# Gaukler/PlainRenderer

Measured on AMD Instinct MI355X. Metric: frames/sec full GI+shade+post @4K; %HBM roofline; 1/2/4/8-GPU scaling, higher is better.
Workload: dtype f32

## Files before the change

### plainrenderer_amd/csrc/backend.cpp

```cpp
#include "backend.h"
#include "kernels_fast/pcf_taps.h"

#include <dlfcn.h>
#include <deque>
#include <algorithm>
#include <chrono>
#include <mutex>
#include <cstdlib>
#include <atomic>
#include <set>
#include <thread>
#include <unordered_map>
#include <unordered_set>
#include <cmath>
#include <cstring>
#include <map>
#include <memory>

#include "../../include/plr.h"

namespace plr {

struct ShaderEntry { std::string name; LaunchFn fn = nullptr; LaunchFn fast = nullptr; };
static bool shaderReadsBindless(const std::string& shader) {
    return shader == "deferredShading.comp" || shader == "sdfDiffuseTrace.comp" || shader == "sdfDebugVisualisation.comp";
}
static bool shaderTakesColumns(const std::string& shader) {
    static const char* const names[] = {"histogramPerTile.comp", "histogramCombineTiles.comp", "depthHiZPyramid.comp", "depthPyramidApex.comp", "depthDownscale.comp",
                                        "sdfCameraTileCulling.comp", "sdfDiffuseTrace.comp", "filterIndirectDiffuseSpatial.comp", "filterIndirectDiffuseTemporal.comp",
                                        "indirectLightUpscale.comp", "deferredShading.comp", "temporalFilter.comp", "bloomDownsample.comp", "bloomUpsample.comp",
                                        "applyBloom.comp", "tonemapping.comp", "giSampleRequests.comp"};
    for (const char* n : names) if (shader == n) return true;
    return false;
}
static bool storageBindingIsReadOnly(const std::string& shader, uint32_t binding) { return shader == "lightMatrix.comp" && binding == 1; }
static std::deque<ShaderEntry>& registry() {
    static std::deque<ShaderEntry> r;
    return r;
}
static std::mutex& registryMutex() {
    static std::mutex m;
    return m;
}
ShaderRegistrar::ShaderRegistrar(const char* name, LaunchFn fn, bool fast) {
    std::lock_guard<std::mutex> lock(registryMutex());
    for (auto& e : registry())
        if (e.name == name) { (fast ? e.fast : e.fn) = fn; return; }
    ShaderEntry e;
    e.name = name;
    (fast ? e.fast : e.fn) = fn;
    registry().push_back(e);
}

struct FusionEntry {
    std::string label;
    std::vector<std::string> shaders;
    FusedLaunchFn fn;
    bool writesSignatures = false;
// ... 1377 lines not shown
        for (size_t k = 0; k < plan.count; k++) { prepareCtx(g->executions[plan.group + k], g->earlyStream, globalPtr); ctxs[k] = &g->executions[plan.group + k].ctx; }
        hipStream_t previous = g->curStream;
        g->curStream = g->earlyStream;
        if (timed) {
            std::string name;
            for (size_t k = 0; k < plan.count; k++) name += (k ? " + " : "") + g->passes[g->executions[plan.group + k].pass]->name;
            name += " (" + plan.f->earlyLabel + ", early stream)";
            if (int trc = beginSegment(g->fusedNames.insert(name).first->c_str())) return trc;
        }
        EarlyPart part;
        part.mode = EarlyPart::Launch;
        const int rc = plan.f->early(ctxs, plan.count, part);
        if (rc) { g_err = "early part of fused launch '" + plan.f->label + "': " + g_err; return rc < 0 ? rc : PLR_ERR_HIP; }
        if (timed) if (int trc = endSegment()) return trc;
        g->curStream = previous;
        if (int erc = orderEvent(&plan.done)) return erc;
        HIP_TRY(hipEventRecord(plan.done, g->earlyStream));
        plan.launched = true;
        g->lastEarly++;
    }
    return PLR_OK;
}

static int tryFusedLaunch(size_t i, size_t last, hipStream_t stream, const GlobalUbo* globalPtr, bool timed, size_t* covered) {
    *covered = 0;
    if (!g->fusion || g->mathMode != PLR_MATH_FAST) return PLR_OK;
    for (const FusionEntry& f : fusions()) {
        const size_t n = f.shaders.size();
        if (i + n > last) continue;
        if (g->debugSig && !f.writesSignatures) continue;
        bool match = true;
        for (size_t k = 0; k < n && match; k++) match = g->passes[g->executions[i + k].pass]->shader == f.shaders[k];
        for (size_t k = 0; k < n && match; k++) match = !g->executions[i + k].edgesFirst();
        if (!match) continue;
        const PassCtx* ctxs[8];
        if (n > 8) continue;
        for (size_t k = 0; k < n; k++) { prepareCtx(g->executions[i + k], stream, globalPtr); ctxs[k] = &g->executions[i + k].ctx; }
        EarlyPlan* early = nullptr;
        for (EarlyPlan& plan : g_earlyPlans) if (plan.launched && plan.group == i && plan.f == &f) early = &plan;
        if (early) {
            HIP_TRY(hipStreamWaitEvent(stream, early->done, 0));
            for (size_t k = 0; k < n; k++) g->executions[i + k].ctx.earlyPartDone = true;
        }
        if (g->fusion >= 2) {
            for (size_t k = 0; k < n; k++) {
                Execution& x = g->executions[i + k];
                for (int b = 0; b < kMaxBindings; b++) {
                    if (!x.ctx.hasStorage(b)) continue;
                    const void* key = nullptr;
                    for (const Access& a : x.access) if (a.write && a.key == x.ctx.storage[b].ptr) key = a.key;
                    if (!key) continue;
                    bool outside = false;
                    for (size_t j = 0; j < g->executions.size() && !outside; j++) {
                        if (j >= i && j < i + n) continue;
                        for (const Access& a : g->executions[j].access) if (a.key == key) { outside = true; break; }
                    }
                    if (!outside) x.ctx.elidableStorage |= 1u << b;
                }
            }
        }
        const char* label = nullptr;
        g->curStream = stream;
        if (timed) {
            std::string name;
            for (size_t k = 0; k < n; k++) name += (k ? " + " : "") + g->passes[g->executions[i + k].pass]->name;
            label = g->fusedNames.insert(name).first->c_str();
            if (int trc = beginSegment(label)) return trc;
        }
        g->currentPassName = label ? label : f.label.c_str();
        for (size_t k = 0; k < n; k++) touchAccesses(g->executions[i + k].access);
        Execution& first = g->executions[i];
        first.ctx.pendingFillSlot = nullptr; first.ctx.pendingFillsTaken = false; first.ctx.applyPendingFillsNow = nullptr;
        if (g->pendingFillSlot) {
            if (f.takesFills && stream == g->stream) { first.ctx.pendingFillSlot = g->pendingFillSlot; first.ctx.applyPendingFillsNow = &applyPendingFillsNow; }
            else if (int frc = applyPendingFillsNow()) return frc;
        }
        for (size_t k = 0; k < n; k++) if (int src = refuseStaleReads(g->executions[i + k], &g->executions[i], n)) return src;
        const int rc = f.fn(ctxs, n);
// ... 678 lines not shown
```

### plainrenderer_amd/csrc/device/image.h

```cpp
#pragma once
#include "vecmath.h"

namespace plr {

enum Format : int32_t {
    F_R8 = 0, F_RG8 = 1, F_RGBA8 = 2, F_R16F = 3, F_RG16F = 4, F_RG32F = 5, F_RG16SN = 6, F_RGBA16F = 7,
    F_RGBA16SN = 8, F_RGBA32F = 9, F_R11G11B10 = 10, F_D16 = 11, F_D32 = 12, F_BC1 = 13, F_BC3 = 14, F_BC5 = 15,
    F_BGRA8 = 16
};

struct ImgView {
    void* ptr;
    int32_t w, h, d;
    int32_t fmt;
};

PLR_DI float halfBitsToFloat(uint32_t h) {
    union { uint16_t u; _Float16 f; } c;
    c.u = (uint16_t)h;
    return (float)c.f;
}
PLR_DI uint32_t floatToHalfBits(float v) {
#ifndef PLR_FAST_SET
    asm volatile("" : "+v"(v));
// ... 18 lines not shown
    const uint32_t subnormal = f2u(v + magic) - f2u(magic);
    uint32_t r = v < 6.103515625e-05f ? subnormal : normal;
    r = r < maxFinite ? r : maxFinite;
    r = u == 0x7f800000u ? expMax : r;
    r = (u >> 31) ? 0u : r;
    r = (u & 0x7fffffffu) > 0x7f800000u ? (expMax | (1u << (M - 1))) : r;
    return r;
}

PLR_DI uint32_t packR11G11B10Exact(vec3 c) {
    return encodeUFloat<6>(c.x) | (encodeUFloat<6>(c.y) << 11) | (encodeUFloat<5>(c.z) << 22);
}

template <int M> PLR_DI uint32_t encodeUFloatInRange(float v) {
    constexpr int shift = 23 - M;
    const uint32_t s = f2u(v * 1.92592994438723585e-34f);
    return (s + ((1u << (shift - 1)) - 1u) + ((s >> shift) & 1u)) >> shift;
}
constexpr uint32_t kUFloatInRangeLimit = 0x477d0000u;
__device__ __attribute__((noinline)) inline uint32_t packR11G11B10OutOfRange(float x, float y, float z) { return packR11G11B10Exact(vec3(x, y, z)); }
PLR_DI uint32_t packR11G11B10Fast(vec3 c) {
    const uint32_t top = max(max(f2u(c.x), f2u(c.y)), f2u(c.z));
    if (__builtin_amdgcn_ballot_w64(top >= kUFloatInRangeLimit) != 0ull) return packR11G11B10OutOfRange(c.x, c.y, c.z);
    return encodeUFloatInRange<6>(c.x) | (encodeUFloatInRange<6>(c.y) << 11) | (encodeUFloatInRange<5>(c.z) << 22);
}

PLR_DI uint32_t packR11G11B10(vec3 c) {
#ifdef PLR_FAST_SET
    return packR11G11B10Fast(c);
#else
    return packR11G11B10Exact(c);
#endif
}

PLR_DI float decodeUnorm8(uint32_t c) { return (float)c / 255.0f; }
PLR_DI float decodeUnorm8Newton(uint32_t c) {
    const float x = (float)c, r = 0x1.010102p-8f, q = x * r;
    return __builtin_fmaf(__builtin_fmaf(-255.f, q, x), r, q);
}
PLR_DI uint32_t encodeUnorm8(float v) {
    if (v != v) return 0u;
    return (uint32_t)__float2int_rn(gclamp(v, 0.f, 1.f) * 255.0f);
}
PLR_DI float decodeSnorm16(int32_t c) { return gmax((float)c / 32767.0f, -1.0f); }
PLR_DI float decodeUnorm16(uint32_t c) { return (float)c / 65535.0f; }

// ... 175 lines not shown
```

### plainrenderer_amd/csrc/kernels_fast/bloom_fast.hip

```cpp
#include "../backend.h"
#include "../device/shading_common.h"
#include <cstdlib>

namespace plr {
namespace fastbloom {

constexpr int TW = 64, TH = 16;
constexpr int ROWS_A = 16, ROWS_B = 12;

struct Tap { int i0, i1; float w0, w1; };

PLR_DI Tap tap1D(float u, int n, float h) {
    int i0; float a;
    linearCoord(u * (float)n, &i0, &a);
    Tap t;
    t.i0 = clampi(i0, n); t.i1 = clampi(i0 + 1, n);
    t.w0 = (1.f - a) * h; t.w1 = a * h;
    return t;
}

template <bool LOWEST>
PLR_DI void bloomUpsampleFastBlock(ImgView source, ImgView previous, ImgView target, float blurRadius, int coverW, int coverH, int yBase, int xBase, unsigned bx, unsigned by) {
    __shared__ float HA[ROWS_A][3][TW];
    __shared__ float HB[ROWS_B][3][TW];
// ... 143 lines not shown
    uint32_t* out = (uint32_t*)target.ptr;
#pragma unroll
    for (int q = 0; q < QY; q++)
#pragma unroll
        for (int py = 0; py < 2; py++) {
            const int y = Y + 2 * q + py;
            if (y >= coverH || y < yBase) continue;
            uint32_t* orow = out + (size_t)y * (size_t)target.w + X;
            const uint32_t p0 = packR11G11B10(acc[q][py][0]), p1 = packR11G11B10(acc[q][py][1]);
            if (X + 1 < coverW) *(uint2*)orow = make_uint2(p0, p1);
            else orow[0] = p0;
        }
}
template <int QY>
__global__ __launch_bounds__(256) void bloomUpsampleQuadKernel(ImgView source, ImgView previous, ImgView target, ParityWeights pw, bool lowest, int coverW, int coverH,
                                                               int yBase, int xBase) { bloomUpsampleQuadBlock<QY>(source, previous, target, pw, lowest, coverW, coverH, yBase, xBase, blockIdx.x, blockIdx.y); }

constexpr int kStripCols = 60, kStripRows = 8;
PLR_DI float laneLeft(float v) { return __builtin_bit_cast(float, __builtin_amdgcn_mov_dpp(__builtin_bit_cast(int, v), 0x138, 0xf, 0xf, true)); }
PLR_DI float laneRight(float v) { return __builtin_bit_cast(float, __builtin_amdgcn_mov_dpp(__builtin_bit_cast(int, v), 0x130, 0xf, 0xf, true)); }
PLR_DI vec3 laneLeft(const vec3& v) { return vec3(laneLeft(v.x), laneLeft(v.y), laneLeft(v.z)); }
PLR_DI vec3 laneRight(const vec3& v) { return vec3(laneRight(v.x), laneRight(v.y), laneRight(v.z)); }

template <bool LOWEST>
__global__ __launch_bounds__(256) void bloomUpsampleStripKernel(ImgView source, ImgView previous, ImgView target, ParityWeights pw, int coverW, int coverH, int yBase, int xBase) {
    const int lane = (int)(threadIdx.x & 63u), wave = (int)(threadIdx.x >> 6);
    const int kc = (xBase >> 1) + (int)blockIdx.x * kStripCols - 2 + lane;
    const int m0 = (yBase >> 1) + ((int)blockIdx.y * 4 + wave) * kStripRows;
    if (2 * m0 >= coverH) return;
    float wt[2][5], wb[2][3];
#pragma unroll
    for (int p = 0; p < 2; p++) {
#pragma unroll
        for (int j = 0; j < 5; j++) { wt[p][j] = pw.tent[p][j]; asm volatile("" : "+v"(wt[p][j])); }
#pragma unroll
        for (int j = 0; j < 3; j++) { wb[p][j] = pw.box[p][j]; asm volatile("" : "+v"(wb[p][j])); }
    }
    const int sw = source.w, sh = source.h;
    const uint32_t* src = (const uint32_t*)source.ptr + clampi(kc, sw);
    uint32_t ta[kStripRows + 4], tb[kStripRows + 2];
#pragma unroll
    for (int r = 0; r < kStripRows + 4; r++) ta[r] = src[(size_t)clampi(m0 - 2 + r, sh) * (size_t)sw];
    if (!LOWEST) {
        const int pwid = previous.w, phei = previous.h;
        const uint32_t* prv = (const uint32_t*)previous.ptr + clampi(kc, pwid);
#pragma unroll
        for (int r = 0; r < kStripRows + 2; r++) tb[r] = prv[(size_t)clampi(m0 - 1 + r, phei) * (size_t)pwid];
    }
    vec3 h0[kStripRows + 4], h1[kStripRows + 4], g0[kStripRows + 2], g1[kStripRows + 2];
    auto tentRow = [&](int r) {
        const vec3 c2 = unpackR11G11B10(ta[r]);
        const vec3 c1 = laneLeft(c2), c0 = laneLeft(c1), c3 = laneRight(c2), c4 = laneRight(c3);
        vec3 a(0.f), b(0.f);
        a = a + c0 * wt[0][0]; b = b + c0 * wt[1][0];
        a = a + c1 * wt[0][1]; b = b + c1 * wt[1][1];
        a = a + c2 * wt[0][2]; b = b + c2 * wt[1][2];
        a = a + c3 * wt[0][3]; b = b + c3 * wt[1][3];
        a = a + c4 * wt[0][4]; b = b + c4 * wt[1][4];
        h0[r] = a; h1[r] = b;
    };
    auto boxRow = [&](int r) {
        const vec3 c1 = unpackR11G11B10(tb[r]);
        const vec3 c0 = laneLeft(c1), c2 = laneRight(c1);
        vec3 a(0.f), b(0.f);
        a = a + c0 * wb[0][0]; b = b + c0 * wb[1][0];
        a = a + c1 * wb[0][1]; b = b + c1 * wb[1][1];
        a = a + c2 * wb[0][2]; b = b + c2 * wb[1][2];
        g0[r] = a; g1[r] = b;
    };
#pragma unroll
    for (int r = 0; r < 4; r++) tentRow(r);
    if (!LOWEST) {
#pragma unroll
        for (int r = 0; r < 2; r++) boxRow(r);
    }
    const bool outputLane = lane >= 2 && lane < 2 + kStripCols && 2 * kc < coverW;
    const bool both = 2 * kc + 1 < coverW;
    uint32_t* out = (uint32_t*)target.ptr + 2 * kc;
#pragma unroll
    for (int q = 0; q < kStripRows; q++) {
        tentRow(q + 4);
        if (!LOWEST) boxRow(q + 2);
#pragma unroll
        for (int py = 0; py < 2; py++) {
            vec3 a(0.f), b(0.f);
#pragma unroll
            for (int j = 0; j < 5; j++) { a = a + h0[q + j] * wt[py][j]; b = b + h1[q + j] * wt[py][j]; }
            if (!LOWEST) {
#pragma unroll
                for (int j = 0; j < 3; j++) { a = a + g0[q + j] * wb[py][j]; b = b + g1[q + j] * wb[py][j]; }
            }
            const int y = 2 * (m0 + q) + py;
            if (y < coverH && outputLane) {
                uint32_t* orow = out + (size_t)y * (size_t)target.w;
                const uint32_t p0 = packR11G11B10(a), p1 = packR11G11B10(b);
                if (both) *(uint2*)orow = make_uint2(p0, p1);
                else orow[0] = p0;
            }
        }
    }
}

static bool accumulateTap(float position, float weight, int base, int n, float* w) {
    const float sane = std::min(std::max(position, -1.0e6f), 1.0e6f);
    const int ti = (int)std::floor((sane - 0.5f) * 256.0f + 0.5f);
    const int i0 = ti >> 8;
    const float a = (float)(ti & 255) * (1.0f / 256.0f);
    const int j0 = i0 - base, j1 = i0 + 1 - base;
    if ((1.f - a) != 0.f) { if (j0 < 0 || j0 >= n) return false; w[j0] += weight * (1.f - a); }
    if (a != 0.f) { if (j1 < 0 || j1 >= n) return false; w[j1] += weight * a; }
    return true;
}

static bool makeParityWeights(float blurRadius, ParityWeights* pw) {
    const int k = 8;
    for (int p = 0; p < 2; p++) {
        const float s = (float)k + 0.25f + 0.5f * (float)p;
        for (float& v : pw->tent[p]) v = 0.f;
        for (float& v : pw->box[p]) v = 0.f;
        bool ok = accumulateTap(s, 0.5f, k - 2, 5, pw->tent[p]) && accumulateTap(s + blurRadius, 0.25f, k - 2, 5, pw->tent[p]) &&
                  accumulateTap(s - blurRadius, 0.25f, k - 2, 5, pw->tent[p]) && accumulateTap(s + 0.5f, 0.5f, k - 1, 3, pw->box[p]) &&
                  accumulateTap(s - 0.5f, 0.5f, k - 1, 3, pw->box[p]);
        if (!ok) return false;
// ... 49 lines not shown
    p.gridX = divUp((unsigned)(w - x0), (unsigned)TW); p.gridY = divUp((unsigned)(h - yBase), (unsigned)TH);
    return 0;
}

static int launch(const PassCtx& c) {
    UpPlan p;
    if (int rc = planUp(c, &p)) return rc;
    const dim3 grid(p.gridX, p.gridY);
    switch (p.kind) {
        case UP_NOTHING: return 0;
        case UP_STRIP:
            if (p.lowest) bloomUpsampleStripKernel<true><<<grid, 256, 0, c.stream>>>(p.source, p.source, p.target, p.pw, p.w, p.h, p.yBase, p.x0);
            else bloomUpsampleStripKernel<false><<<grid, 256, 0, c.stream>>>(p.source, p.previous, p.target, p.pw, p.w, p.h, p.yBase, p.x0);
            break;
        case UP_QUAD: bloomUpsampleQuadKernel<kQuadQY><<<grid, 256, 0, c.stream>>>(p.source, p.previous, p.target, p.pw, p.lowest != 0, p.w, p.h, p.yBase, p.x0); break;
        default:
            if (p.lowest) bloomUpsampleFastKernel<true><<<grid, 256, 0, c.stream>>>(p.source, p.source, p.target, p.blurRadius, p.w, p.h, p.yBase, p.x0);
            else bloomUpsampleFastKernel<false><<<grid, 256, 0, c.stream>>>(p.source, p.previous, p.target, p.blurRadius, p.w, p.h, p.yBase, p.x0);
    }
    PLR_CHECK_LAUNCH(c);
    return 0;
}

PLR_DI void bloomDownsampleFastBlock(ImgView source, ImgView target, int coverW, int coverH, int yBase, int xBase, unsigned bx, unsigned by) {
    const int k = (xBase >> 1) + (int)(bx * 64u + (threadIdx.x & 63u));
    const int m = (yBase >> 1) + (int)(by * 4u + (threadIdx.x >> 6));
    const int X = 2 * k, Y = 2 * m;
    if (X >= coverW || Y >= coverH) return;
    const uint32_t* src = (const uint32_t*)source.ptr;
    const int sx = 4 * k - 1;
    const bool interior = sx >= 0 && sx + 5 < source.w;
    vec3 centre[2][2], border[2][2];
#pragma unroll
    for (int i = 0; i < 4; i++) { centre[i >> 1][i & 1] = vec3(0.f); border[i >> 1][i & 1] = vec3(0.f); }
#pragma unroll
    for (int r = 0; r < 6; r++) {
        const uint32_t* row = src + (size_t)clampi(4 * m - 1 + r, source.h) * (size_t)source.w;
        uint32_t t[6];
        if (interior) {
            uint4 v; uint2 u;
            __builtin_memcpy(&v, row + sx, 16);
            __builtin_memcpy(&u, row + sx + 4, 8);
            t[0] = v.x; t[1] = v.y; t[2] = v.z; t[3] = v.w; t[4] = u.x; t[5] = u.y;
        } else { for (int c = 0; c < 6; c++) t[c] = row[clampi(sx + c, source.w)]; }
        vec3 col[6];
#pragma unroll
// ... 199 lines not shown
            L.source = d.source; L.previous = d.source; L.target = d.target; L.blurRadius = 0.f; L.lowest = 0;
            L.w = d.w; L.h = d.h; L.yBase = d.y0; L.x0 = d.x0; L.kind = d.kind; L.gridX = d.gridX; L.tiles = d.gridX * d.gridY;
        }
        if (L.tiles == 0 || (int)L.tiles > chainMaxTiles()) return kUseGeneralKernel;
        if (i > 0 && L.source.ptr != cp.level[i - 1].target.ptr) return kUseGeneralKernel;
        maxTiles = std::max(maxTiles, L.tiles);
    }
    const PassCtx& c = *ctxs[0];
    cp.counters = (uint32_t*)c.scratch(64);
    if (!cp.counters) return kUseGeneralKernel;
    unsigned grid = 0;
    if (int rc = chainGrid<UP>(c, maxTiles, &grid)) return rc;
    bloomChainKernel<UP><<<grid, 256, 0, c.stream>>>(cp);
    PLR_CHECK_LAUNCH(c);
    return 0;
}

}

static int fastbloom_up_launch(const PassCtx& c) { return fastbloom::launch(c); }
PLR_REGISTER_SHADER_FAST("bloomUpsample.comp", fastbloom_up_launch);
static int fastbloom_down_launch(const PassCtx& c) { return fastbloom::launchDown(c); }
PLR_REGISTER_SHADER_FAST("bloomDownsample.comp", fastbloom_down_launch);
static int fastbloom_down_chain(const PassCtx* const* ctxs, size_t count) { return fastbloom::launchChain<false>(ctxs, count); }
static int fastbloom_up_chain(const PassCtx* const* ctxs, size_t count) { return fastbloom::launchChain<true>(ctxs, count); }
static int fastbloom_down_chain4(const PassCtx* const* ctxs, size_t count) { return fastbloom_down_chain(ctxs, count); }
static int fastbloom_down_chain3(const PassCtx* const* ctxs, size_t count) { return fastbloom_down_chain(ctxs, count); }
static int fastbloom_down_chain2(const PassCtx* const* ctxs, size_t count) { return fastbloom_down_chain(ctxs, count); }
static int fastbloom_up_chain4(const PassCtx* const* ctxs, size_t count) { return fastbloom_up_chain(ctxs, count); }
static int fastbloom_up_chain3(const PassCtx* const* ctxs, size_t count) { return fastbloom_up_chain(ctxs, count); }
static int fastbloom_up_chain2(const PassCtx* const* ctxs, size_t count) { return fastbloom_up_chain(ctxs, count); }
PLR_REGISTER_FUSION("bloomDownsample x4 (persistent chain)", fastbloom_down_chain4, "bloomDownsample.comp", "bloomDownsample.comp", "bloomDownsample.comp", "bloomDownsample.comp");
PLR_REGISTER_FUSION("bloomDownsample x3 (persistent chain)", fastbloom_down_chain3, "bloomDownsample.comp", "bloomDownsample.comp", "bloomDownsample.comp");
PLR_REGISTER_FUSION("bloomDownsample x2 (persistent chain)", fastbloom_down_chain2, "bloomDownsample.comp", "bloomDownsample.comp");
PLR_REGISTER_FUSION("bloomUpsample x4 (persistent chain)", fastbloom_up_chain4, "bloomUpsample.comp", "bloomUpsample.comp", "bloomUpsample.comp", "bloomUpsample.comp");
PLR_REGISTER_FUSION("bloomUpsample x3 (persistent chain)", fastbloom_up_chain3, "bloomUpsample.comp", "bloomUpsample.comp", "bloomUpsample.comp");
PLR_REGISTER_FUSION("bloomUpsample x2 (persistent chain)", fastbloom_up_chain2, "bloomUpsample.comp", "bloomUpsample.comp");
}
```

### plainrenderer_amd/csrc/kernels_fast/gi_spatial_fast.hip

```cpp
#include "../backend.h"
#include "../device/shading_common.h"
#include "../device/xcd.h"
#include "../device/buffer_fetch.h"
#include "fused_gi.h"
#include <cstdlib>
#include <map>
#include <utility>
#include <vector>
#include <type_traits>

namespace plr {

PLR_DI float rcpf(float x) { return __builtin_amdgcn_rcpf(x); }

constexpr int kSampleKeys = 5, kSampleTableFloats = 160;
__global__ void spatialSampleTableKernel(float* __restrict__ table) {
    const int key = (int)threadIdx.x / 32, i = (int)threadIdx.x % 32;
    if (key >= kSampleKeys) return;
    uint32_t rngState = wang_hash((uint32_t)key);
    float r0 = 0.f, r1 = 0.f;
    for (int k = 0; k <= i; k++) { r0 = rand01(rngState); r1 = rand01(rngState); }
    float sn, cs;
    det_sincosf(2.f * PLR_GLSL_PI * r1, &sn, &cs);
    float* t = table + key * kSampleTableFloats;
// ... 32 lines not shown
    if (wi >= words) return;
    uint8_t* bytes = blockIdx.y ? bytes1 : bytes0;
    uint32_t* bitmap = blockIdx.y ? bitmap1 : bitmap0;
    const uint32_t y = wi / rowWords, xw = wi - y * rowWords;
    uint4* src = (uint4*)(bytes + (size_t)y * pitch + (size_t)xw * 32u);
    const uint4 a = src[0], c = src[1];
    const uint32_t d[8] = {a.x, a.y, a.z, a.w, c.x, c.y, c.z, c.w};
    uint32_t bits = 0u;
#pragma unroll
    for (int k = 0; k < 8; k++) {
        const uint32_t v = d[k];
        bits |= (((v & 0xffu) ? 1u : 0u) | ((v & 0xff00u) ? 2u : 0u) | ((v & 0xff0000u) ? 4u : 0u) | ((v & 0xff000000u) ? 8u : 0u)) << (4 * k);
    }
    bitmap[wi] = bits;
    if (bits) { src[0] = make_uint4(0u, 0u, 0u, 0u); src[1] = make_uint4(0u, 0u, 0u, 0u); }
}

struct SpatialFrameConsts {
    float tsx, tsy;
    float dW, dH;
    float nW, nH;
    float3 vpRowNorms;
};
template <int DEPTH_FMT, int TX, bool SAME_GRID, bool PACKED, bool SIG, bool MARK = false>
__global__ __launch_bounds__(256) void spatialFilterFastKernel(ImgView outYSH, ImgView outCoCg, ImgView inYSH, ImgView inCoCg, ImgView depthTexture, ImgView normalTexture,
                                                               const GlobalUbo* __restrict__ g, const float* __restrict__ sampleTables, const uint4* __restrict__ packed, int filterIndex,
                                                               int coverW, int coverH, int yBase, int xBase, int tilesX, int tilesY, int chunkRows, uint32_t* __restrict__ sig,
                                                               uint32_t validY0, uint32_t validRowCount, uint32_t validX0, uint32_t validColCount, int rowMissShrinks,
                                                               SpatialFrameConsts fc, uint32_t* __restrict__ requestBitmap = nullptr, uint32_t bitmapRowWords = 0, int requestPhase = 0,
                                                               uint32_t* __restrict__ requestBitmap2 = nullptr) {
    const float* samples = sampleTables + min(g->frameIndexMod4 + (uint32_t)filterIndex, (uint32_t)(kSampleKeys - 1)) * kSampleTableFloats;
    constexpr int TY = 256 / TX;
    int tileX, tileY;
    if (!xcdWalk2(tilesX, tilesY, chunkRows & 0xffff, chunkRows >> 16, tileX, tileY)) return;
    const int px = xBase + tileX * TX + (int)(threadIdx.x % TX);
    const int py = yBase + tileY * TY + (int)(threadIdx.x / TX);
    if (px >= coverW || py >= coverH) return;

    const float nearP = g->nearPlane, farP = g->farPlane;
    const float nf = nearP * farP, nmf = nearP - farP;
    const vec3 fwd = ld3(g->cameraForward), up = ld3(g->cameraUp), right = ld3(g->cameraRight), camPos = ld3(g->cameraPosition);
    const float tanH = g->cameraTanFovHalf, tanA = g->cameraTanFovHalf * g->cameraAspectRatio;
    const float dW = fc.dW, dH = fc.dH;
    const int dwi = depthTexture.w, dhi = depthTexture.h;

    float radiusWorld = filterIndex == 1 ? 1.f : 1.5f;
    if (MARK || requestPhase != 0) {
        const uint32_t rY0 = MARK ? validY0 : (uint32_t)yBase, rYn = MARK ? validRowCount : (uint32_t)(coverH - yBase);
// ... 481 lines not shown
```

### plainrenderer_amd/csrc/kernels_fast/stream_fast.hip

```cpp
#include "../backend.h"
#include "../device/shading_common.h"
#include "fused_gi.h"
#include "upscale_quad.h"
#include "../device/fastmath.h"

namespace plr {
namespace faststream {

PLR_DI float rcpf(float x) { return __builtin_amdgcn_rcpf(x); }
PLR_DI float clamp01(float x) { return __builtin_amdgcn_fmed3f(x, 0.f, 1.f); }

__global__ __launch_bounds__(256) void applyBloomFastKernel(ImgView target, ImgView bloom, float strength, int coverW, int coverH, int yBase, int xBase) {
    const int x0 = xBase + (int)(blockIdx.x * 64u + (threadIdx.x & 63u)) * 4;
    const int y = yBase + (int)(blockIdx.y * 4u + (threadIdx.x >> 6));
    if (y >= coverH || x0 >= coverW) return;
    uint32_t* trow = (uint32_t*)target.ptr + (size_t)y * (size_t)target.w;
    const uint32_t* brow = (const uint32_t*)bloom.ptr + (size_t)y * (size_t)bloom.w;
    const int n = min(4, coverW - x0);
    uint32_t s[4] = {0u, 0u, 0u, 0u}, b[4] = {0u, 0u, 0u, 0u};
    const bool wide = n == 4 && (target.w & 3) == 0;
    if (wide) {
        const uint4 sv = *(const uint4*)(trow + x0), bv = *(const uint4*)(brow + x0);
        s[0] = sv.x; s[1] = sv.y; s[2] = sv.z; s[3] = sv.w; b[0] = bv.x; b[1] = bv.y; b[2] = bv.z; b[3] = bv.w;
    } else for (int i = 0; i < n; i++) { s[i] = trow[x0 + i]; b[i] = brow[x0 + i]; }
    uint32_t o[4];
#pragma unroll
    for (int i = 0; i < 4; i++) {
        const vec3 sc = unpackR11G11B10(s[i]), bc = unpackR11G11B10(b[i]);
        o[i] = packR11G11B10(sc + (bc - sc) * strength);
    }
    if (wide) *(uint4*)(trow + x0) = make_uint4(o[0], o[1], o[2], o[3]);
    else for (int i = 0; i < n; i++) trow[x0 + i] = o[i];
}

static int launchApplyBloom(const PassCtx& c) {
    if (int rc = c.needStorage(0, F_R11G11B10, "applyBloom target")) return rc;
    if (int rc = c.needSampled(1, F_R11G11B10, "applyBloom bloomTexture")) return rc;
    if (c.push.size() < 4) return c.fail(-1, "applyBloom: push constant bloomStrength missing");
    const ImgView& target = c.storage[0];
    if (c.sampled[1].w != target.w || c.sampled[1].h != target.h) return kUseGeneralKernel;
    float strength;
    std::memcpy(&strength, c.push.data(), 4);
    const PassCtx::RowSpan rs = c.rowSpan(target.h);
    const PassCtx::ColSpan cs = c.colSpan(target.w);
    const int w = cs.x1, x0 = cs.x0, h = rs.y1, y0 = rs.y0;
    if (w <= x0 || h <= y0) return 0;
    applyBloomFastKernel<<<dim3(divUp((unsigned)(w - x0), 256u), divUp((unsigned)(h - y0), 4u)), 256, 0, c.stream>>>(target, c.sampled[1], strength, w, h, y0, x0);
    PLR_CHECK_LAUNCH(c);
    return 0;
}

PLR_DI float srgb(float l) {
    const float hi = __builtin_amdgcn_exp2f((1.0f / 2.4f) * __builtin_amdgcn_logf(fabsf(l))) * 1.055f - 0.055f;
    return l <= 0.0031308f ? l * 12.92f : hi;
}
PLR_DI uint32_t unorm8(float v) { return (uint32_t)__float2int_rn(clamp01(v) * 255.0f); }

template <bool BGRA>
PLR_DI uint32_t tonemapPixel(vec3 c, int x, float time, uint32_t nyA, uint32_t nyB) {
    const uint32_t UI0 = 1597334673u, UI1 = 3812015801u, UI2 = 2798796415u;
    const float UIF = 1.0f / (float)0xffffffffu;
    vec3 v(0.59719f * c.x + 0.35458f * c.y + 0.04823f * c.z, 0.07600f * c.x + 0.90834f * c.y + 0.01566f * c.z, 0.02840f * c.x + 0.13383f * c.y + 0.83777f * c.z);
    const vec3 a = v * (v + 0.0245786f) - 0.000090537f;
    const vec3 b = v * (0.983729f * v + 0.4329510f) + 0.238081f;
    v = vec3(a.x * rcpf(b.x), a.y * rcpf(b.y), a.z * rcpf(b.z));
    const vec3 o(clamp01(1.60475f * v.x + -0.53108f * v.y + -0.07367f * v.z), clamp01(-0.10208f * v.x + 1.10813f * v.y + -0.00605f * v.z),
                 clamp01(-0.00327f * v.x + -0.07276f * v.y + 1.07602f * v.z));
    const uint32_t qxA = (uint32_t)(int32_t)(float)(uint32_t)((float)x * time), qxB = (uint32_t)(int32_t)(float)(uint32_t)(((float)x + 165.f) * time);
    const uint32_t mA = (qxA * UI0) ^ nyA ^ (qxA * UI2), mB = (qxB * UI0) ^ nyB ^ (qxB * UI2);
    const vec3 noise = (vec3((float)(mA * UI0), (float)(mA * UI1), (float)(mA * UI2)) + vec3((float)(mB * UI0), (float)(mB * UI1), (float)(mB * UI2))) * UIF - 1.f;
    const vec3 s = vec3(srgb(o.x), srgb(o.y), srgb(o.z)) + noise * (1.f / 255.f);
    uint32_t p = unorm8(s.z) | (unorm8(s.y) << 8) | (unorm8(s.x) << 16) | (255u << 24);
    if (!BGRA) p = (p & 0xff00ff00u) | ((p >> 16) & 0xffu) | ((p & 0xffu) << 16);
    return p;
}
PLR_DI void tonemapRowTerms(int y, float time, uint32_t* nyA, uint32_t* nyB) {
    const uint32_t UI1 = 3812015801u;
    const uint32_t qyA = (uint32_t)(int32_t)(float)(uint32_t)((float)y * time), qyB = (uint32_t)(int32_t)(float)(uint32_t)(((float)y + 1292.f) * time);
    *nyA = qyA * UI1; *nyB = qyB * UI1;
}

template <bool BGRA>
__global__ __launch_bounds__(256) void tonemappingFastKernel(ImgView src, ImgView dst, const GlobalUbo* __restrict__ g, int coverW, int coverH, int yBase, int xBase) {
    const int x0 = xBase + (int)(blockIdx.x * 64u + (threadIdx.x & 63u)) * 4;
    const int y = yBase + (int)(blockIdx.y * 4u + (threadIdx.x >> 6));
    if (y >= coverH || x0 >= coverW) return;
    const float time = g->time;
    const uint32_t* srow = (const uint32_t*)src.ptr + (size_t)y * (size_t)src.w;
    uint32_t* drow = (uint32_t*)dst.ptr + (size_t)y * (size_t)dst.w;
    const int n = min(4, coverW - x0);
    uint32_t in[4] = {0u, 0u, 0u, 0u}, out[4];
    const bool wide = n == 4 && (src.w & 3) == 0 && (dst.w & 3) == 0;
    if (wide) { const uint4 v = *(const uint4*)(srow + x0); in[0] = v.x; in[1] = v.y; in[2] = v.z; in[3] = v.w; }
    else for (int i = 0; i < n; i++) in[i] = srow[x0 + i];
    uint32_t nyA, nyB;
    tonemapRowTerms(y, time, &nyA, &nyB);
#pragma unroll
    for (int i = 0; i < 4; i++) out[i] = tonemapPixel<BGRA>(unpackR11G11B10(in[i]), x0 + i, time, nyA, nyB);
    if (wide) *(uint4*)(drow + x0) = make_uint4(out[0], out[1], out[2], out[3]);
    else for (int i = 0; i < n; i++) drow[x0 + i] = out[i];
}

template <bool BGRA>
__global__ __launch_bounds__(256) void applyBloomTonemapKernel(ImgView target, ImgView bloom, ImgView dst, const GlobalUbo* __restrict__ g, float strength, int coverW, int coverH, int yBase, int xBase) {
    const int x0 = xBase + (int)(blockIdx.x * 64u + (threadIdx.x & 63u)) * 4;
    const int y = yBase + (int)(blockIdx.y * 4u + (threadIdx.x >> 6));
    if (y >= coverH || x0 >= coverW) return;
    const float time = g->time;
    uint32_t* trow = (uint32_t*)target.ptr + (size_t)y * (size_t)target.w;
    const uint32_t* brow = (const uint32_t*)bloom.ptr + (size_t)y * (size_t)bloom.w;
    uint32_t* drow = (uint32_t*)dst.ptr + (size_t)y * (size_t)dst.w;
    const uint4 sv = *(const uint4*)(trow + x0), bv = *(const uint4*)(brow + x0);
    const uint32_t s[4] = {sv.x, sv.y, sv.z, sv.w}, b[4] = {bv.x, bv.y, bv.z, bv.w};
    uint32_t nyA, nyB;
    tonemapRowTerms(y, time, &nyA, &nyB);
    uint32_t o[4], t[4];
#pragma unroll
    for (int i = 0; i < 4; i++) {
        const vec3 sc = unpackR11G11B10(s[i]), bc = unpackR11G11B10(b[i]);
        o[i] = packR11G11B10(sc + (bc - sc) * strength);
        t[i] = tonemapPixel<BGRA>(unpackR11G11B10(o[i]), x0 + i, time, nyA, nyB);
    }
    *(uint4*)(trow + x0) = make_uint4(o[0], o[1], o[2], o[3]);
    *(uint4*)(drow + x0) = make_uint4(t[0], t[1], t[2], t[3]);
}

static int launchTonemapping(const PassCtx& c) {
    if (int rc = c.needGlobal()) return rc;
    if (int rc = c.needSampled(1, F_R11G11B10, "tonemapping imageIn")) return rc;
    if (int rc = c.needStorage(0, -1, "tonemapping imageOut")) return rc;
    const ImgView& src = c.sampled[1];
    const ImgView& dst = c.storage[0];
    if (dst.fmt != F_BGRA8 && dst.fmt != F_RGBA8) return c.fail(-4, "tonemapping imageOut must be BGRA8_uNorm or RGBA8");
    const PassCtx::ColSpan cs = c.colSpan(std::min(dst.w, src.w));
    const int coverW = cs.x1, xBase = cs.x0;
    const PassCtx::RowSpan rs = c.rowSpan(std::min(dst.h, src.h));
    const int coverH = rs.y1, y0 = rs.y0;
    if (coverW <= xBase || coverH <= y0) return 0;
    const dim3 grid(divUp((unsigned)(coverW - xBase), 256u), divUp((unsigned)(coverH - y0), 4u));
    if (dst.fmt == F_BGRA8) tonemappingFastKernel<true><<<grid, 256, 0, c.stream>>>(src, dst, c.global, coverW, coverH, y0, xBase);
    else tonemappingFastKernel<false><<<grid, 256, 0, c.stream>>>(src, dst, c.global, coverW, coverH, y0, xBase);
    PLR_CHECK_LAUNCH(c);
    return 0;
}

struct Pair8 { uint2 a, b; };
PLR_DI Pair8 loadPairRGBA16F(const ImgView& im, int x0, int x1, int y) {
// ... 377 lines not shown
```

Before: 1426.

## Fuse final bloom upsample with applyBloom and tonemapping into one strip kernel

Adds a fusion that runs the mip-0 bloom upsample, the bloom apply and tonemapping in a single strip kernel. The upsampled bloom is exchanged between lane pairs via DPP and consumed directly, so the full-resolution bloom target write can be skipped when nothing else reads it, which removes one full-res write plus two reads and two launches. Elision analysis now checks per-mip bindings for bloom shaders, and per-column dither terms are precomputed in LDS. The fused kernel carries higher register pressure, pins waves_per_eu and prefetches rows, which could cost occupancy.

```diff
diff --git a/plainrenderer_amd/csrc/backend.cpp b/plainrenderer_amd/csrc/backend.cpp
--- a/plainrenderer_amd/csrc/backend.cpp
+++ b/plainrenderer_amd/csrc/backend.cpp
@@ -34,6 +34,7 @@
     return false;
 }
 static bool storageBindingIsReadOnly(const std::string& shader, uint32_t binding) { return shader == "lightMatrix.comp" && binding == 1; }
+static bool shaderAddressesBoundMipsOnly(const std::string& shader) { return shader == "bloomDownsample.comp" || shader == "bloomUpsample.comp"; }
 static std::deque<ShaderEntry>& registry() {
     static std::deque<ShaderEntry> r;
     return r;
@@ -1457,6 +1458,16 @@
     return PLR_OK;
 }
 
+static bool touchesLevel(const Execution& y, const void* key, const ImgView& level) {
+    bool names = false;
+    for (const Access& a : y.access) names = names || a.key == key;
+    if (!names) return false;
+    if (y.callback || !shaderAddressesBoundMipsOnly(g->passes[y.pass]->shader)) return true;
+    for (int b = 0; b < kMaxBindings; b++)
+        if ((y.ctx.hasSampled(b) && y.ctx.sampled[b].ptr == level.ptr) || (y.ctx.hasStorage(b) && y.ctx.storage[b].ptr == level.ptr)) return true;
+    return false;
+}
+
 static int tryFusedLaunch(size_t i, size_t last, hipStream_t stream, const GlobalUbo* globalPtr, bool timed, size_t* covered) {
     *covered = 0;
     if (!g->fusion || g->mathMode != PLR_MATH_FAST) return PLR_OK;
@@ -1488,7 +1499,7 @@
                     bool outside = false;
                     for (size_t j = 0; j < g->executions.size() && !outside; j++) {
                         if (j >= i && j < i + n) continue;
-                        for (const Access& a : g->executions[j].access) if (a.key == key) { outside = true; break; }
+                        outside = touchesLevel(g->executions[j], key, x.ctx.storage[b]);
                     }
                     if (!outside) x.ctx.elidableStorage |= 1u << b;
                 }
diff --git a/plainrenderer_amd/csrc/device/image.h b/plainrenderer_amd/csrc/device/image.h
--- a/plainrenderer_amd/csrc/device/image.h
+++ b/plainrenderer_amd/csrc/device/image.h
@@ -64,6 +64,11 @@
 PLR_DI uint32_t packR11G11B10Fast(vec3 c) {
     const uint32_t top = max(max(f2u(c.x), f2u(c.y)), f2u(c.z));
     if (__builtin_amdgcn_ballot_w64(top >= kUFloatInRangeLimit) != 0ull) return packR11G11B10OutOfRange(c.x, c.y, c.z);
+    return encodeUFloatInRange<6>(c.x) | (encodeUFloatInRange<6>(c.y) << 11) | (encodeUFloatInRange<5>(c.z) << 22);
+}
+PLR_DI uint32_t packR11G11B10FastInline(vec3 c) {
+    const uint32_t top = max(max(f2u(c.x), f2u(c.y)), f2u(c.z));
+    if (__builtin_expect(__builtin_amdgcn_ballot_w64(top >= kUFloatInRangeLimit) != 0ull, 0)) return packR11G11B10Exact(c);
     return encodeUFloatInRange<6>(c.x) | (encodeUFloatInRange<6>(c.y) << 11) | (encodeUFloatInRange<5>(c.z) << 22);
 }
 
diff --git a/plainrenderer_amd/csrc/kernels_fast/bloom_fast.hip b/plainrenderer_amd/csrc/kernels_fast/bloom_fast.hip
--- a/plainrenderer_amd/csrc/kernels_fast/bloom_fast.hip
+++ b/plainrenderer_amd/csrc/kernels_fast/bloom_fast.hip
@@ -1,5 +1,6 @@
 #include "../backend.h"
 #include "../device/shading_common.h"
+#include "tonemap_pixel.h"
 #include <cstdlib>
 
 namespace plr {
@@ -189,8 +190,17 @@
 PLR_DI vec3 laneLeft(const vec3& v) { return vec3(laneLeft(v.x), laneLeft(v.y), laneLeft(v.z)); }
 PLR_DI vec3 laneRight(const vec3& v) { return vec3(laneRight(v.x), laneRight(v.y), laneRight(v.z)); }
 
-template <bool LOWEST>
-__global__ __launch_bounds__(256) void bloomUpsampleStripKernel(ImgView source, ImgView previous, ImgView target, ParityWeights pw, int coverW, int coverH, int yBase, int xBase) {
+PLR_DI uint32_t lanePartner(uint32_t v) { return (uint32_t)__builtin_amdgcn_mov_dpp((int)v, 0xB1, 0xf, 0xf, true); }
+
+struct StripTail {
+    ImgView scene, dst;
+    const GlobalUbo* global;
+    float strength;
+    int storeLevel;
+};
+
+template <bool LOWEST, int TAIL>
+PLR_DI void bloomUpsampleStripBody(ImgView source, ImgView previous, ImgView target, ParityWeights pw, int coverW, int coverH, int yBase, int xBase, const StripTail& tail) {
     const int lane = (int)(threadIdx.x & 63u), wave = (int)(threadIdx.x >> 6);
     const int kc = (xBase >> 1) + (int)blockIdx.x * kStripCols - 2 + lane;
     const int m0 = (yBase >> 1) + ((int)blockIdx.y * 4 + wave) * kStripRows;
@@ -205,16 +215,21 @@
     }
     const int sw = source.w, sh = source.h;
     const uint32_t* src = (const uint32_t*)source.ptr + clampi(kc, sw);
+    constexpr int kTailAhead = 1;
+    constexpr int aheadA = TAIL ? 4 + kTailAhead : kStripRows + 4, aheadB = TAIL ? 2 + kTailAhead : kStripRows + 2;
     uint32_t ta[kStripRows + 4], tb[kStripRows + 2];
-#pragma unroll
-    for (int r = 0; r < kStripRows + 4; r++) ta[r] = src[(size_t)clampi(m0 - 2 + r, sh) * (size_t)sw];
+    const int pwid = previous.w, phei = previous.h;
+    const uint32_t* prv = (const uint32_t*)previous.ptr + clampi(kc, pwid);
+    auto loadA = [&](int r) { ta[r] = src[(size_t)clampi(m0 - 2 + r, sh) * (size_t)sw]; };
+    auto loadB = [&](int r) { tb[r] = prv[(size_t)clampi(m0 - 1 + r, phei) * (size_t)pwid]; };
+#pragma unroll
+    for (int r = 0; r < aheadA; r++) loadA(r);
     if (!LOWEST) {
-        const int pwid = previous.w, phei = previous.h;
-        const uint32_t* prv = (const uint32_t*)previous.ptr + clampi(kc, pwid);
-#pragma unroll
-        for (int r = 0; r < kStripRows + 2; r++) tb[r] = prv[(size_t)clampi(m0 - 1 + r, phei) * (size_t)pwid];
+#pragma unroll
+        for (int r = 0; r < aheadB; r++) loadB(r);
     }
     vec3 h0[kStripRows + 4], h1[kStripRows + 4], g0[kStripRows + 2], g1[kStripRows + 2];
+    auto pin = [](vec3& a, vec3& b) { asm volatile("" : "+v"(a.x), "+v"(a.y), "+v"(a.z), "+v"(b.x), "+v"(b.y), "+v"(b.z)); };
     auto tentRow = [&](int r) {
         const vec3 c2 = unpackR11G11B10(ta[r]);
         const vec3 c1 = laneLeft(c2), c0 = laneLeft(c1), c3 = laneRight(c2), c4 = laneRight(c3);
@@ -224,6 +239,7 @@
         a = a + c2 * wt[0][2]; b = b + c2 * wt[1][2];
         a = a + c3 * wt[0][3]; b = b + c3 * wt[1][3];
         a = a + c4 * wt[0][4]; b = b + c4 * wt[1][4];
+        if (TAIL) pin(a, b);
         h0[r] = a; h1[r] = b;
     };
     auto boxRow = [&](int r) {
@@ -233,6 +249,7 @@
         a = a + c0 * wb[0][0]; b = b + c0 * wb[1][0];
         a = a + c1 * wb[0][1]; b = b + c1 * wb[1][1];
         a = a + c2 * wb[0][2]; b = b + c2 * wb[1][2];
+        if (TAIL) pin(a, b);
         g0[r] = a; g1[r] = b;
     };
 #pragma unroll
@@ -244,10 +261,31 @@
     const bool outputLane = lane >= 2 && lane < 2 + kStripCols && 2 * kc < coverW;
     const bool both = 2 * kc + 1 < coverW;
     uint32_t* out = (uint32_t*)target.ptr + 2 * kc;
+    const int odd = lane & 1, x4 = 2 * (kc - odd);
+    const bool tailLane = lane >= 2 && lane < 2 + kStripCols && x4 + 3 < coverW;
+    __shared__ uint32_t columnTerms[4][8][64];
+    float time = 0.f;
+    if (TAIL) {
+        time = tail.global->time;
+#pragma unroll
+        for (int i = 0; i < 4; i++) {
+            uint32_t nxA, nxB;
+            faststream::tonemapColumnTerms(x4 + i, time, &nxA, &nxB);
+            columnTerms[wave][i][lane] = nxA; columnTerms[wave][4 + i][lane] = nxB;
+        }
+    }
 #pragma unroll
     for (int q = 0; q < kStripRows; q++) {
+        const int yt = 2 * (m0 + q) + odd;
+        uint4 sv = make_uint4(0u, 0u, 0u, 0u);
+        if (TAIL) sv = *(const uint4*)((const uint32_t*)tail.scene.ptr + (size_t)min(yt, coverH - 1) * (size_t)tail.scene.w + min(max(x4, 0), coverW - 4));
+        if (TAIL) {
+            if (q + aheadA < kStripRows + 4) loadA(q + aheadA);
+            if (!LOWEST && q + aheadB < kStripRows + 2) loadB(q + aheadB);
+        }
         tentRow(q + 4);
         if (!LOWEST) boxRow(q + 2);
+        uint32_t packed[2][2];
 #pragma unroll
         for (int py = 0; py < 2; py++) {
             vec3 a(0.f), b(0.f);
@@ -257,6 +295,7 @@
 #pragma unroll
                 for (int j = 0; j < 3; j++) { a = a + g0[q + j] * wb[py][j]; b = b + g1[q + j] * wb[py][j]; }
             }
+            if (TAIL) { packed[py][0] = packR11G11B10FastInline(a); packed[py][1] = packR11G11B10FastInline(b); continue; }
             const int y = 2 * (m0 + q) + py;
             if (y < coverH && outputLane) {
                 uint32_t* orow = out + (size_t)y * (size_t)target.w;
@@ -265,7 +304,33 @@
                 else orow[0] = p0;
             }
         }
-    }
+        if (TAIL) {
+            const uint32_t r0 = lanePartner(odd ? packed[0][0] : packed[1][0]), r1 = lanePartner(odd ? packed[0][1] : packed[1][1]);
+            const uint4 bv = odd ? make_uint4(r0, r1, packed[1][0], packed[1][1]) : make_uint4(packed[0][0], packed[0][1], r0, r1);
+            if (yt < coverH && tailLane) {
+                const size_t o = (size_t)yt * (size_t)tail.scene.w + x4;
+                if (tail.storeLevel) *(uint4*)((uint32_t*)target.ptr + o) = bv;
+                uint32_t nyA, nyB;
+                faststream::tonemapRowTerms(yt, time, &nyA, &nyB);
+                int slot = lane;
+                asm volatile("" : "+v"(slot));
+                uint4 applied, shown;
+                faststream::applyBloomTonemap4<TAIL == 1, true>(sv, bv, tail.strength,
+                                                                [&](int i, uint32_t* nxA, uint32_t* nxB) { *nxA = columnTerms[wave][i][slot]; *nxB = columnTerms[wave][4 + i][slot]; },
+                                                                nyA, nyB, &applied, &shown);
+                *(uint4*)((uint32_t*)tail.scene.ptr + o) = applied;
+                *(uint4*)((uint32_t*)tail.dst.ptr + o) = shown;
+            }
+        }
+    }
+}
+template <bool LOWEST>
+__global__ __launch_bounds__(256) void bloomUpsampleStripKernel(ImgView source, ImgView previous, ImgView target, ParityWeights pw, int coverW, int coverH, int yBase, int xBase) {
+    bloomUpsampleStripBody<LOWEST, 0>(source, previous, target, pw, coverW, coverH, yBase, xBase, StripTail{});
+}
+template <bool BGRA>
+__global__ __launch_bounds__(256) __attribute__((amdgpu_waves_per_eu(5))) void bloomUpsampleApplyTonemapKernel(ImgView source, ImgView previous, ImgView target, ParityWeights pw, int coverW, int coverH, int yBase, int xBase, StripTail tail) {
+    bloomUpsampleStripBody<false, BGRA ? 1 : 2>(source, previous, target, pw, coverW, coverH, yBase, xBase, tail);
 }
 
 static bool accumulateTap(float position, float weight, int base, int n, float* w) {
@@ -361,6 +426,37 @@
     return 0;
 }
 
+static int launchStripTail(const PassCtx* const* ctxs, size_t count) {
+    if (count != 3) return kUseGeneralKernel;
+    const PassCtx &u = *ctxs[0], &a = *ctxs[1], &t = *ctxs[2];
+    if (!u.hasStorage(0) || !u.hasSampled(1) || !u.hasSampled(2) || u.push.size() < 4 || u.specBool(0, false)) return kUseGeneralKernel;
+    if (u.storage[0].fmt != F_R11G11B10 || u.sampled[1].fmt != F_R11G11B10 || u.sampled[2].fmt != F_R11G11B10) return kUseGeneralKernel;
+    if (!a.hasStorage(0) || !a.hasSampled(1) || !t.hasStorage(0) || !t.hasSampled(1) || !t.global || a.push.size() < 4) return kUseGeneralKernel;
+    const ImgView &scene = a.storage[0], &bloom = a.sampled[1], &src = t.sampled[1], &dst = t.storage[0];
+    if (scene.fmt != F_R11G11B10 || bloom.fmt != F_R11G11B10 || (dst.fmt != F_BGRA8 && dst.fmt != F_RGBA8)) return kUseGeneralKernel;
+    if (src.ptr != scene.ptr || src.w != scene.w || src.h != scene.h) return kUseGeneralKernel;
+    if (bloom.ptr != u.storage[0].ptr || bloom.w != u.storage[0].w || bloom.h != u.storage[0].h) return kUseGeneralKernel;
+    if (bloom.w != scene.w || bloom.h != scene.h || dst.w != scene.w || dst.h != scene.h || (scene.w & 3)) return kUseGeneralKernel;
+    if (scene.ptr == bloom.ptr || dst.ptr == bloom.ptr || dst.ptr == scene.ptr || u.sampled[1].ptr == scene.ptr || u.sampled[2].ptr == scene.ptr) return kUseGeneralKernel;
+    UpPlan p;
+    if (planUp(u, &p) != 0 || p.kind != UP_STRIP || p.lowest) return kUseGeneralKernel;
+    const PassCtx::RowSpan ra = a.rowSpan(scene.h), rt = t.rowSpan(scene.h);
+    const PassCtx::ColSpan ca = a.colSpan(scene.w), ct = t.colSpan(scene.w);
+    if (ra.y0 != rt.y0 || ra.y1 != rt.y1 || ca.x0 != ct.x0 || ca.x1 != ct.x1 || ra.y0 != p.yBase || ra.y1 != p.h || ca.x0 != p.x0 || ca.x1 != p.w) return kUseGeneralKernel;
+    if (((ca.x1 - ca.x0) & 3) || (ca.x0 & 7)) return kUseGeneralKernel;
+    StripTail tail;
+    tail.scene = scene; tail.dst = dst; tail.global = t.global;
+    std::memcpy(&tail.strength, a.push.data(), 4);
+    const bool elide = (u.elidableStorage & 1u) != 0;
+    tail.storeLevel = elide ? 0 : 1;
+    const dim3 grid(p.gridX, p.gridY);
+    if (dst.fmt == F_BGRA8) bloomUpsampleApplyTonemapKernel<true><<<grid, 256, 0, u.stream>>>(p.source, p.previous, p.target, p.pw, p.w, p.h, p.yBase, p.x0, tail);
+    else bloomUpsampleApplyTonemapKernel<false><<<grid, 256, 0, u.stream>>>(p.source, p.previous, p.target, p.pw, p.w, p.h, p.yBase, p.x0, tail);
+    PLR_CHECK_LAUNCH(u);
+    if (elide) u.elidedStorage = 1u;
+    return 0;
+}
+
 PLR_DI void bloomDownsampleFastBlock(ImgView source, ImgView target, int coverW, int coverH, int yBase, int xBase, unsigned bx, unsigned by) {
     const int k = (xBase >> 1) + (int)(bx * 64u + (threadIdx.x & 63u));
     const int m = (yBase >> 1) + (int)(by * 4u + (threadIdx.x >> 6));
@@ -606,6 +702,8 @@
 PLR_REGISTER_SHADER_FAST("bloomUpsample.comp", fastbloom_up_launch);
 static int fastbloom_down_launch(const PassCtx& c) { return fastbloom::launchDown(c); }
 PLR_REGISTER_SHADER_FAST("bloomDownsample.comp", fastbloom_down_launch);
+static int fastbloom_strip_tail(const PassCtx* const* ctxs, size_t count) { return fastbloom::launchStripTail(ctxs, count); }
+PLR_REGISTER_FUSION("bloomUpsample mip 0 + applyBloom + tonemapping", fastbloom_strip_tail, "bloomUpsample.comp", "applyBloom.comp", "tonemapping.comp");
 static int fastbloom_down_chain(const PassCtx* const* ctxs, size_t count) { return fastbloom::launchChain<false>(ctxs, count); }
 static int fastbloom_up_chain(const PassCtx* const* ctxs, size_t count) { return fastbloom::launchChain<true>(ctxs, count); }
 static int fastbloom_down_chain4(const PassCtx* const* ctxs, size_t count) { return fastbloom_down_chain(ctxs, count); }
diff --git a/plainrenderer_amd/csrc/kernels_fast/gi_spatial_fast.hip b/plainrenderer_amd/csrc/kernels_fast/gi_spatial_fast.hip
--- a/plainrenderer_amd/csrc/kernels_fast/gi_spatial_fast.hip
+++ b/plainrenderer_amd/csrc/kernels_fast/gi_spatial_fast.hip
@@ -78,8 +78,11 @@
     float nW, nH;
     float3 vpRowNorms;
 };
+#ifndef PLR_SPATIAL_OCC
+#define PLR_SPATIAL_OCC
+#endif
 template <int DEPTH_FMT, int TX, bool SAME_GRID, bool PACKED, bool SIG, bool MARK = false>
-__global__ __launch_bounds__(256) void spatialFilterFastKernel(ImgView outYSH, ImgView outCoCg, ImgView inYSH, ImgView inCoCg, ImgView depthTexture, ImgView normalTexture,
+__global__ __launch_bounds__(256) PLR_SPATIAL_OCC void spatialFilterFastKernel(ImgView outYSH, ImgView outCoCg, ImgView inYSH, ImgView inCoCg, ImgView depthTexture, ImgView normalTexture,
                                                                const GlobalUbo* __restrict__ g, const float* __restrict__ sampleTables, const uint4* __restrict__ packed, int filterIndex,
                                                                int coverW, int coverH, int yBase, int xBase, int tilesX, int tilesY, int chunkRows, uint32_t* __restrict__ sig,
                                                                uint32_t validY0, uint32_t validRowCount, uint32_t validX0, uint32_t validColCount, int rowMissShrinks,
diff --git a/plainrenderer_amd/csrc/kernels_fast/stream_fast.hip b/plainrenderer_amd/csrc/kernels_fast/stream_fast.hip
--- a/plainrenderer_amd/csrc/kernels_fast/stream_fast.hip
+++ b/plainrenderer_amd/csrc/kernels_fast/stream_fast.hip
@@ -3,12 +3,10 @@
 #include "fused_gi.h"
 #include "upscale_quad.h"
 #include "../device/fastmath.h"
+#include "tonemap_pixel.h"
 
 namespace plr {
 namespace faststream {
-
-PLR_DI float rcpf(float x) { return __builtin_amdgcn_rcpf(x); }
-PLR_DI float clamp01(float x) { return __builtin_amdgcn_fmed3f(x, 0.f, 1.f); }
 
 __global__ __launch_bounds__(256) void applyBloomFastKernel(ImgView target, ImgView bloom, float strength, int coverW, int coverH, int yBase, int xBase) {
     const int x0 = xBase + (int)(blockIdx.x * 64u + (threadIdx.x & 63u)) * 4;
@@ -48,36 +46,6 @@
     applyBloomFastKernel<<<dim3(divUp((unsigned)(w - x0), 256u), divUp((unsigned)(h - y0), 4u)), 256, 0, c.stream>>>(target, c.sampled[1], strength, w, h, y0, x0);
     PLR_CHECK_LAUNCH(c);
     return 0;
-}
-
-PLR_DI float srgb(float l) {
-    const float hi = __builtin_amdgcn_exp2f((1.0f / 2.4f) * __builtin_amdgcn_logf(fabsf(l))) * 1.055f - 0.055f;
-    return l <= 0.0031308f ? l * 12.92f : hi;
-}
-PLR_DI uint32_t unorm8(float v) { return (uint32_t)__float2int_rn(clamp01(v) * 255.0f); }
-
-template <bool BGRA>
-PLR_DI uint32_t tonemapPixel(vec3 c, int x, float time, uint32_t nyA, uint32_t nyB) {
-    const uint32_t UI0 = 1597334673u, UI1 = 3812015801u, UI2 = 2798796415u;
-    const float UIF = 1.0f / (float)0xffffffffu;
-    vec3 v(0.59719f * c.x + 0.35458f * c.y + 0.04823f * c.z, 0.07600f * c.x + 0.90834f * c.y + 0.01566f * c.z, 0.02840f * c.x + 0.13383f * c.y + 0.83777f * c.z);
-    const vec3 a = v * (v + 0.0245786f) - 0.000090537f;
-    const vec3 b = v * (0.983729f * v + 0.4329510f) + 0.238081f;
-    v = vec3(a.x * rcpf(b.x), a.y * rcpf(b.y), a.z * rcpf(b.z));
-    const vec3 o(clamp01(1.60475f * v.x + -0.53108f * v.y + -0.07367f * v.z), clamp01(-0.10208f * v.x + 1.10813f * v.y + -0.00605f * v.z),
-                 clamp01(-0.00327f * v.x + -0.07276f * v.y + 1.07602f * v.z));
-    const uint32_t qxA = (uint32_t)(int32_t)(float)(uint32_t)((float)x * time), qxB = (uint32_t)(int32_t)(float)(uint32_t)(((float)x + 165.f) * time);
-    const uint32_t mA = (qxA * UI0) ^ nyA ^ (qxA * UI2), mB = (qxB * UI0) ^ nyB ^ (qxB * UI2);
-    const vec3 noise = (vec3((float)(mA * UI0), (float)(mA * UI1), (float)(mA * UI2)) + vec3((float)(mB * UI0), (float)(mB * UI1), (float)(mB * UI2))) * UIF - 1.f;
-    const vec3 s = vec3(srgb(o.x), srgb(o.y), srgb(o.z)) + noise * (1.f / 255.f);
-    uint32_t p = unorm8(s.z) | (unorm8(s.y) << 8) | (unorm8(s.x) << 16) | (255u << 24);
-    if (!BGRA) p = (p & 0xff00ff00u) | ((p >> 16) & 0xffu) | ((p & 0xffu) << 16);
-    return p;
-}
-PLR_DI void tonemapRowTerms(int y, float time, uint32_t* nyA, uint32_t* nyB) {
-    const uint32_t UI1 = 3812015801u;
-    const uint32_t qyA = (uint32_t)(int32_t)(float)(uint32_t)((float)y * time), qyB = (uint32_t)(int32_t)(float)(uint32_t)(((float)y + 1292.f) * time);
-    *nyA = qyA * UI1; *nyB = qyB * UI1;
 }
 
 template <bool BGRA>
@@ -111,18 +79,12 @@
     const uint32_t* brow = (const uint32_t*)bloom.ptr + (size_t)y * (size_t)bloom.w;
     uint32_t* drow = (uint32_t*)dst.ptr + (size_t)y * (size_t)dst.w;
     const uint4 sv = *(const uint4*)(trow + x0), bv = *(const uint4*)(brow + x0);
-    const uint32_t s[4] = {sv.x, sv.y, sv.z, sv.w}, b[4] = {bv.x, bv.y, bv.z, bv.w};
     uint32_t nyA, nyB;
     tonemapRowTerms(y, time, &nyA, &nyB);
-    uint32_t o[4], t[4];
-#pragma unroll
-    for (int i = 0; i < 4; i++) {
-        const vec3 sc = unpackR11G11B10(s[i]), bc = unpackR11G11B10(b[i]);
-        o[i] = packR11G11B10(sc + (bc - sc) * strength);
-        t[i] = tonemapPixel<BGRA>(unpackR11G11B10(o[i]), x0 + i, time, nyA, nyB);
-    }
-    *(uint4*)(trow + x0) = make_uint4(o[0], o[1], o[2], o[3]);
-    *(uint4*)(drow + x0) = make_uint4(t[0], t[1], t[2], t[3]);
+    uint4 o, t;
+    applyBloomTonemap4<BGRA>(sv, bv, strength, [&](int i, uint32_t* nxA, uint32_t* nxB) { tonemapColumnTerms(x0 + i, time, nxA, nxB); }, nyA, nyB, &o, &t);
+    *(uint4*)(trow + x0) = o;
+    *(uint4*)(drow + x0) = t;
 }
 
 static int launchTonemapping(const PassCtx& c) {
diff --git a/plainrenderer_amd/csrc/kernels_fast/tonemap_pixel.h b/plainrenderer_amd/csrc/kernels_fast/tonemap_pixel.h
--- /dev/null
+++ b/plainrenderer_amd/csrc/kernels_fast/tonemap_pixel.h
@@ -0,0 +1,69 @@
+#pragma once
+#include "../device/shading_common.h"
+
+namespace plr {
+namespace faststream {
+
+PLR_DI float rcpf(float x) { return __builtin_amdgcn_rcpf(x); }
+PLR_DI float clamp01(float x) { return __builtin_amdgcn_fmed3f(x, 0.f, 1.f); }
+
+PLR_DI float srgb(float l) {
+    const float hi = __builtin_amdgcn_exp2f((1.0f / 2.4f) * __builtin_amdgcn_logf(fabsf(l))) * 1.055f - 0.055f;
+    return l <= 0.0031308f ? l * 12.92f : hi;
+}
+PLR_DI uint32_t unorm8(float v) { return (uint32_t)__float2int_rn(clamp01(v) * 255.0f); }
+
+PLR_DI void tonemapColumnTerms(int x, float time, uint32_t* nxA, uint32_t* nxB) {
+    const uint32_t UI0 = 1597334673u, UI2 = 2798796415u;
+    const uint32_t qxA = (uint32_t)(int32_t)(float)(uint32_t)((float)x * time), qxB = (uint32_t)(int32_t)(float)(uint32_t)(((float)x + 165.f) * time);
+    *nxA = (qxA * UI0) ^ (qxA * UI2); *nxB = (qxB * UI0) ^ (qxB * UI2);
+}
+PLR_DI void tonemapRowTerms(int y, float time, uint32_t* nyA, uint32_t* nyB) {
+    const uint32_t UI1 = 3812015801u;
+    const uint32_t qyA = (uint32_t)(int32_t)(float)(uint32_t)((float)y * time), qyB = (uint32_t)(int32_t)(float)(uint32_t)(((float)y + 1292.f) * time);
+    *nyA = qyA * UI1; *nyB = qyB * UI1;
+}
+
+template <bool BGRA>
+PLR_DI uint32_t tonemapPixel(vec3 c, uint32_t nxA, uint32_t nxB, uint32_t nyA, uint32_t nyB) {
+    const uint32_t UI0 = 1597334673u, UI1 = 3812015801u, UI2 = 2798796415u;
+    const float UIF = 1.0f / (float)0xffffffffu;
+    vec3 v(0.59719f * c.x + 0.35458f * c.y + 0.04823f * c.z, 0.07600f * c.x + 0.90834f * c.y + 0.01566f * c.z, 0.02840f * c.x + 0.13383f * c.y + 0.83777f * c.z);
+    const vec3 a = v * (v + 0.0245786f) - 0.000090537f;
+    const vec3 b = v * (0.983729f * v + 0.4329510f) + 0.238081f;
+    v = vec3(a.x * rcpf(b.x), a.y * rcpf(b.y), a.z * rcpf(b.z));
+    const vec3 o(clamp01(1.60475f * v.x + -0.53108f * v.y + -0.07367f * v.z), clamp01(-0.10208f * v.x + 1.10813f * v.y + -0.00605f * v.z),
+                 clamp01(-0.00327f * v.x + -0.07276f * v.y + 1.07602f * v.z));
+    const uint32_t mA = nxA ^ nyA, mB = nxB ^ nyB;
+    const vec3 noise = (vec3((float)(mA * UI0), (float)(mA * UI1), (float)(mA * UI2)) + vec3((float)(mB * UI0), (float)(mB * UI1), (float)(mB * UI2))) * UIF - 1.f;
+    const vec3 s = vec3(srgb(o.x), srgb(o.y), srgb(o.z)) + noise * (1.f / 255.f);
+    uint32_t p = unorm8(s.z) | (unorm8(s.y) << 8) | (unorm8(s.x) << 16) | (255u << 24);
+    if (!BGRA) p = (p & 0xff00ff00u) | ((p >> 16) & 0xffu) | ((p & 0xffu) << 16);
+    return p;
+}
+template <bool BGRA>
+PLR_DI uint32_t tonemapPixel(vec3 c, int x, float time, uint32_t nyA, uint32_t nyB) {
+    uint32_t nxA, nxB;
+    tonemapColumnTerms(x, time, &nxA, &nxB);
+    return tonemapPixel<BGRA>(c, nxA, nxB, nyA, nyB);
+}
+
+template <bool BGRA, bool INLINE_PACK = false, typename ColumnTerms>
+PLR_DI void applyBloomTonemap4(const uint4 sv, const uint4 bv, float strength, ColumnTerms columnTerms, uint32_t nyA, uint32_t nyB, uint4* applied, uint4* tonemapped) {
+    const uint32_t s[4] = {sv.x, sv.y, sv.z, sv.w}, b[4] = {bv.x, bv.y, bv.z, bv.w};
+    uint32_t o[4], t[4];
+#pragma unroll
+    for (int i = 0; i < 4; i++) {
+        const vec3 sc = unpackR11G11B10(s[i]), bc = unpackR11G11B10(b[i]);
+        const vec3 mixed = sc + (bc - sc) * strength;
+        o[i] = INLINE_PACK ? packR11G11B10FastInline(mixed) : packR11G11B10(mixed);
+        uint32_t nxA, nxB;
+        columnTerms(i, &nxA, &nxB);
+        t[i] = tonemapPixel<BGRA>(unpackR11G11B10(o[i]), nxA, nxB, nyA, nyB);
+    }
+    *applied = make_uint4(o[0], o[1], o[2], o[3]);
+    *tonemapped = make_uint4(t[0], t[1], t[2], t[3]);
+}
+
+}
+}
```

New measurement: 1420. No clear change (-0.4%).
